# PNP-team/ZPrize23-gpu-submission

Measured on AMD Instinct MI355X. Metric: gen_proof wall-clock (s), HEIGHT=15 Poseidon tree, 1/2/4/8 MI355X + HBM GB/s, lower is better.
Workload: dtype u64

## Files before the change

### zprize23-gpu-submission_amd/csrc/msm.hip

```cpp
#include <algorithm>
#include "msm_internal.h"
#include "ec.cuh"
#include "ec29.cuh"

namespace pnp {

constexpr uint32_t KEY_ZERO = 0xFFFFFFFFu;
template <int C, class E>
__device__ __forceinline__ void digits_of(const Fr &s, int c_rt, int W_rt, int top_sh, E emit) {
    const int c = C > 0 ? C : c_rt;
    const int W = C > 0 ? (255 + C) / C : W_rt;
    const uint32_t NB = 1u << (c - 1);
    uint32_t carry = 0;
    auto digit = [&](int w) {
        const int bit = w * c;
        const int li = bit >> 5, sh = bit & 31;
        uint32_t lo32 = 0, hi32 = 0;
#pragma unroll
        for (int k = 0; k < 8; k++) {
            lo32 = li == k ? s.v[k] : lo32;
            hi32 = li + 1 == k ? s.v[k] : hi32;
        }
        const uint64_t word = lo32 | ((uint64_t)hi32 << 32);
        uint32_t raw = (uint32_t)(word >> sh) & ((1u << c) - 1);
        raw += carry;
        uint32_t key = KEY_ZERO;
        if (raw > NB) {
            const uint32_t mag = (NB << 1) - raw;
            carry = 1;
            if (mag) key = (mag - 1) | 0x80000000u;
        } else {
            carry = 0;
            if (raw) key = (w == W - 1 ? raw << top_sh : raw) - 1;
        }
        emit(w, key);
    };
    if constexpr (C > 0) {
#pragma unroll
        for (int w = 0; w < (255 + C) / C; w++) digit(w);
    } else {
        for (int w = 0; w < W; w++) digit(w);
    }
}
template <class F>
__device__ __forceinline__ void scalar_digits(const uint64_t *scalars, uint64_t i, uint64_t n, int c, int W,
                                              int top_sh, uint32_t *keys, F fn) {
    const Fr s = from_mont(load_fr(scalars, i));
    auto emit = [&](int w, uint32_t key) {
        keys[(uint64_t)w * n + i] = key;
        fn(key);
    };
    if (c == 20 && W == 13)
        digits_of<20>(s, c, W, top_sh, emit);
    else
        digits_of<0>(s, c, W, top_sh, emit);
}
__global__ void k_digits(const uint64_t *scalars, uint64_t n, int c, int W, int top_sh, uint32_t *keys) {
    uint64_t i = blockIdx.x * (uint64_t)blockDim.x + threadIdx.x;
    if (i >= n) return;
    scalar_digits(scalars, i, n, c, W, top_sh, keys, [](uint32_t) {});
}

constexpr int MSM_BATCH_MAX = 16;
struct KeyRows {
    uint64_t n;
    int vstride, off, rows;
    uint32_t id_row0;
    uint64_t id_mul;
    uint64_t id_base = 0;
    int nseg = 0;
    uint64_t seg_off[MSM_BATCH_MAX] = {};
};

#ifndef PNP_SORT_CB
#define PNP_SORT_CB 9
#endif
constexpr int SORT_CB = PNP_SORT_CB;
constexpr int SORT_FB_MAX = 11;
static_assert(SORT_CB >= 1 && SORT_CB <= 12, "PNP_SORT_CB out of range (LDS budget of k_coarse_scatter)");
__device__ __forceinline__ uint64_t cidx(int v, int nv, uint32_t b, int NBc, int wmaj, int ch, int nch) {
    if (wmaj <= 1) return ((uint64_t)v * NBc + b) * nch + ch;
    const uint32_t nbl = (uint32_t)NBc / wmaj;
    return (((uint64_t)(b / nbl) * nv + v) * nbl + b % nbl) * nch + ch;
}

__global__ __launch_bounds__(1024) void k_coarse_hist(const uint32_t *keys, KeyRows kr, int fb,
                                                      int NBc, uint64_t chunk, int nch,
                                                      uint32_t *counts, int wmaj = 1) {
    __shared__ uint32_t hist[1 << SORT_CB];
    const int v = blockIdx.y, ch = blockIdx.x;
    for (int b = threadIdx.x; b < NBc; b += blockDim.x) hist[b] = 0;
    __syncthreads();
    const uint64_t n = kr.n;
    uint64_t lo = (uint64_t)ch * chunk, hi = lo + chunk < n ? lo + chunk : n;
    const uint32_t *kb = keys + ((uint64_t)v * kr.vstride + kr.off) * n;
    const bool vec = ((n | chunk) & 3) == 0;
    for (int r = 0; r < kr.rows; r++) {
        const uint32_t *k = kb + (uint64_t)r * n;
        if (vec) {
            for (uint64_t i = lo + 4 * threadIdx.x; i < hi; i += 4 * blockDim.x) {
                uint4 q = *reinterpret_cast<const uint4 *>(k + i);
                uint32_t w[4] = {q.x, q.y, q.z, q.w};
#pragma unroll
                for (int j = 0; j < 4; j++)
                    if (w[j] != KEY_ZERO) atomicAdd(&hist[(w[j] & 0x7FFFFFFFu) >> fb], 1u);
            }
        } else {
            for (uint64_t i = lo + threadIdx.x; i < hi; i += blockDim.x) {
                uint32_t key = k[i];
                if (key != KEY_ZERO) atomicAdd(&hist[(key & 0x7FFFFFFFu) >> fb], 1u);
            }
        }
    }
    __syncthreads();
    for (int b = threadIdx.x; b < NBc; b += blockDim.x) counts[cidx(v, gridDim.y, b, NBc, wmaj, ch, nch)] = hist[b];
}

struct ScalarPtrs {
    static constexpr int MAX = MSM_BATCH_MAX;
    const uint64_t *p[MAX];
};
__global__ __launch_bounds__(1024) void k_digits_hist(ScalarPtrs sp, uint64_t n, int c, int W, int top_sh, int fb,
                                                      int NBc,
                                                      uint64_t chunk, int nch, uint32_t *keys, uint32_t *counts,
                                                      int wmaj = 1) {
    __shared__ uint32_t hist[1 << SORT_CB];
    const int v = blockIdx.y, ch = blockIdx.x;
    for (int b = threadIdx.x; b < NBc; b += blockDim.x) hist[b] = 0;
    __syncthreads();
    const uint64_t lo = (uint64_t)ch * chunk, hi = lo + chunk < n ? lo + chunk : n;
    uint32_t *kv = keys + (uint64_t)v * W * n;
    for (uint64_t i = lo + threadIdx.x; i < hi; i += blockDim.x)
        scalar_digits(sp.p[v], i, n, c, W, top_sh, kv, [&](uint32_t key) {
            if (key != KEY_ZERO) atomicAdd(&hist[(key & 0x7FFFFFFFu) >> fb], 1u);
        });
    __syncthreads();
    for (int b = threadIdx.x; b < NBc; b += blockDim.x) counts[cidx(v, gridDim.y, b, NBc, wmaj, ch, nch)] = hist[b];
}

__global__ __launch_bounds__(256) void k_scan_tiles(uint32_t *d, uint64_t n, uint32_t *tile_sums) {
    __shared__ uint32_t wsum[4];
    uint64_t base = (uint64_t)blockIdx.x * 1024;
    uint32_t v[4], loc = 0;
    for (int k = 0; k < 4; k++) {
        uint64_t i = base + threadIdx.x * 4 + k;
        v[k] = i < n ? d[i] : 0;
        loc += v[k];
    }
    uint32_t x = loc;
    int lane = threadIdx.x & 63, wv = threadIdx.x >> 6;
    for (int off = 1; off < 64; off <<= 1) {
        uint32_t y = __shfl_up(x, off, 64);
        if (lane >= off) x += y;
    }
    if (lane == 63) wsum[wv] = x;
    __syncthreads();
// ... 346 lines not shown
    const uint32_t d = blockIdx.x;
    auto bin_off = [&](uint64_t gbin) { return offs[gbin * nch]; };
    uint32_t over = 0;
    for (int e = 0; e < W; e++) over |= bin_off((uint64_t)(e + 1) * per_d) - bin_off((uint64_t)e * per_d) > cap;
    uint32_t *h = reinterpret_cast<uint32_t *>(send + (uint64_t)d * slot_recs);
    const uint64_t g0 = (uint64_t)d * per_d;
    if (threadIdx.x == 0) {
        h[0] = SLOT_MAGIC;
        h[1] = bin_off(g0 + per_d) - bin_off(g0);
        h[2] = over;
        h[3] = per_d;
        if (dest_counts) dest_counts[d] = h[1];
    }
    for (uint32_t p = threadIdx.x; p < per_d; p += blockDim.x) h[4 + p] = bin_off(g0 + p + 1) - bin_off(g0 + p);
}

__device__ uint32_t block_scan_1024(uint32_t x, uint32_t &excl, uint32_t *wsum) {
    const int lane = threadIdx.x & 63, wv = threadIdx.x >> 6;
    uint32_t inc = x;
    for (int off = 1; off < 64; off <<= 1) {
        const uint32_t y = __shfl_up(inc, off, 64);
        if (lane >= off) inc += y;
    }
    if (lane == 63) wsum[wv] = inc;
    __syncthreads();
    uint32_t pre = 0, tot = 0;
    for (int j = 0; j < 16; j++) {
        pre += j < wv ? wsum[j] : 0;
        tot += wsum[j];
    }
    excl = pre + inc - x;
    __syncthreads();
    return tot;
}

constexpr int SLOT_W_MAX = 64;
__global__ __launch_bounds__(1024) void k_slot_runs(const uint64_t *recv, int W, uint32_t slot_recs,
                                                    uint32_t hdr_recs, uint32_t per_d, uint32_t cap, uint2 *runs,
                                                    uint32_t *out0, uint32_t *bstart_end, uint32_t *flags) {
    __shared__ uint32_t wsum[16];
    __shared__ uint32_t rcarry[SLOT_W_MAX];
    __shared__ uint32_t bad;
    if (threadIdx.x == 0) bad = 0;
    if (threadIdx.x < (uint32_t)W) rcarry[threadIdx.x] = 0;
    __syncthreads();
    if (threadIdx.x < (uint32_t)W) {
        const uint32_t *h = reinterpret_cast<const uint32_t *>(recv + (uint64_t)threadIdx.x * slot_recs);
        if (h[0] != SLOT_MAGIC || h[3] != per_d || h[2]) atomicOr(&bad, 1u);
    }
    __syncthreads();
    uint32_t carry = 0;
    for (uint32_t p0 = 0; p0 < per_d; p0 += 1024) {
        const uint32_t p = p0 + threadIdx.x;
        uint32_t sum = 0;
        for (int r = 0; r < W; r++) {
            const uint32_t *h = reinterpret_cast<const uint32_t *>(recv + (uint64_t)r * slot_recs);
            const uint32_t c = p < per_d ? h[4 + p] : 0;
            uint32_t pre;
            const uint32_t tot = block_scan_1024(c, pre, wsum);
            const uint32_t st = rcarry[r] + pre;
            const uint32_t len = st >= cap ? 0 : (c < cap - st ? c : cap - st);
            if (p < per_d) runs[(uint64_t)p * W + r] = make_uint2((uint32_t)r * slot_recs + hdr_recs + st, len);
            sum += len;
            __syncthreads();
            if (threadIdx.x == 0) rcarry[r] += tot;
        }
        uint32_t pre;
        const uint32_t tot = block_scan_1024(sum, pre, wsum);
        if (p < per_d) out0[p] = carry + pre;
        carry += tot;
    }
    if (threadIdx.x == 0) {
        out0[per_d] = carry;
        bstart_end[0] = carry;
        flags[0] = bad;
        flags[1] = carry;
    }
}

__device__ __forceinline__ uint32_t bucket_start(const uint32_t *offs, uint64_t u, int nch) {
    return offs[u * nch];
}
__device__ __forceinline__ uint64_t next_bucket(const uint32_t *offs, int nch, uint64_t U, uint64_t a, uint32_t k,
                                                uint32_t &next) {
    uint64_t lo = a, hi = a + 1, step = 1;
    uint32_t vhi = bucket_start(offs, hi, nch);
    while (vhi <= k) {
        lo = hi;
        step <<= 1;
        hi = lo + step < U ? lo + step : U;
        vhi = bucket_start(offs, hi, nch);
    }
    while (hi - lo > 1) {
        const uint64_t m = (lo + hi) >> 1;
        const uint32_t vm = bucket_start(offs, m, nch);
        if (vm <= k) lo = m;
        else hi = m, vhi = vm;
    }
    next = vhi;
    return lo;
}
template <class LoadPt, class StorePt>
__device__ __forceinline__ void segment32(uint64_t t, LoadPt ld, StorePt st, const uint32_t *sorted,
                                          const uint32_t *offs, int nch, uint64_t U, uint32_t S) {
    const uint32_t total = bucket_start(offs, U, nch);
    const uint64_t lo64 = t * S;
    if (lo64 >= total) return;
    const uint32_t lo = (uint32_t)lo64;
    const uint32_t hi = lo + S < total ? lo + S : total;
    uint64_t a = 0, b = U;
    while (b - a > 1) {
        uint64_t m = (a + b) >> 1;
        if (bucket_start(offs, m, nch) <= lo) a = m; else b = m;
    }
    uint64_t cur = a;
    bool first = bucket_start(offs, cur, nch) < lo;
    uint32_t next = bucket_start(offs, cur + 1, nch);
    Xyzz acc = Xyzz::inf();
    for (uint32_t k = lo; k < hi; k++) {
        if (k == next) {
            if (first) st(1, t, acc);
            else st(0, cur, acc);
            first = false;
            acc = Xyzz::inf();
            cur = next_bucket(offs, nch, U, cur + 1, k, next);
        }
        uint32_t e = sorted[k];
        Fq x, y;
        ld(e & 0x7FFFFFFFu, x, y);
        if (e >> 31) y = neg(y);
        acc = madd(acc, x, y);
    }
    if (first) st(1, t, acc);
    else if (next > hi) st(2, t, acc);
    else st(0, cur, acc);
}

__global__ __launch_bounds__(256) void k_accumulate_flat(const uint64_t *points,
                                                         const uint32_t *sorted,
                                                         const uint32_t *offs, int nch, uint64_t U,
                                                         uint32_t S, uint64_t *buckets,
                                                         uint64_t *head, uint64_t *tail) {
    uint64_t t = blockIdx.x * (uint64_t)blockDim.x + threadIdx.x;
    auto ld = [points](uint32_t i, Fq &x, Fq &y) {
        x = load_fq(points + 12ULL * i);
        y = load_fq(points + 12ULL * i + 6);
    };
    auto st = [=](int where, uint64_t i, const Xyzz &p) {
        store_xyzz((where == 0 ? buckets : where == 1 ? head : tail) + 24 * i, p);
    };
    segment32(t, ld, st, sorted, offs, nch, U, S);
}

__device__ __forceinline__ void madd29(Xyzz29 &p, const F29 &x2, const F29 &y2) {
    F29 u2 = mul29(x2, p.zz);
    F29 s2 = mul29(y2, p.zzz);
    F29 P = sub29(u2, p.x, F29_KB);
    F29 R = sub29(s2, p.y, F29_KB);
    F29 pp = sqr29(P);
    F29 ppp = mul29(P, pp);
    F29 q = mul29(p.x, pp);
    F29 x3 = sub29(sub29(sub29(sqr29(R), ppp, F29_KA), q, F29_KA), q, F29_KA);
    F29 y3 = mul2_29(R, sub29(q, x3, F29_KB), p.y, neg29(ppp, F29_KA));
    p.zz = mul29(p.zz, pp);
    p.zzz = mul29(p.zzz, ppp);
    p.x = x3;
    p.y = y3;
}
__device__ __forceinline__ bool store29(uint32_t *dst, const Xyzz29 &p) {
    store_f29(dst, p.x);
    store_f29(dst + 14, p.y);
    store_f29(dst + 28, p.zz);
    store_f29(dst + 42, p.zzz);
    return !zero29(p.zz);
}

#ifndef PNP_ACC_WAVES
#define PNP_ACC_WAVES 3
#endif
#ifndef PNP_PT29
#define PNP_PT29 32
#endif
static constexpr uint64_t PT29 = PNP_PT29;

typedef __attribute__((address_space(3))) void lds_void_t;
typedef __attribute__((address_space(1))) void glob_void_t;
__device__ __forceinline__ void stage_point(const uint32_t *p, uint4 *st) {
#pragma unroll
    for (int c = 0; c < 7; c++)
        __builtin_amdgcn_global_load_lds((glob_void_t *)(p + 4 * c), (lds_void_t *)(st + 64 * c), 16, 0, 0);
}
__device__ __forceinline__ void unstage_point(const uint4 *st, F29 &x, F29 &y) {
    uint32_t w[28];
#pragma unroll
    for (int c = 0; c < 7; c++) {
        const uint4 v = st[64 * c];
        w[4 * c] = v.x;
        w[4 * c + 1] = v.y;
        w[4 * c + 2] = v.z;
        w[4 * c + 3] = v.w;
    }
#pragma unroll
    for (int i = 0; i < 14; i++) {
        x.l[i] = w[i];
        y.l[i] = w[14 + i];
    }
}

__global__ __launch_bounds__(256, PNP_ACC_WAVES) void k_accumulate29(const uint32_t *pts29, const uint32_t *sorted,
                                                      const uint32_t *offs, uint64_t U, uint32_t S,
                                                      uint32_t *buckets, uint32_t *head,
                                                      uint32_t *tail, uint32_t *tailb, uint32_t *redo,
                                                      uint32_t *nredo, uint32_t *tlist) {
    __shared__ uint4 stage[4 * 7 * 64];
    __shared__ uint32_t sidx[4 * 64];
    const uint32_t wv = threadIdx.x >> 6, ln = threadIdx.x & 63;
    uint4 *wave_base = stage + 7 * 64 * wv;
    uint32_t *idx_base = sidx + 64 * wv;
    uint64_t t = blockIdx.x * (uint64_t)blockDim.x + threadIdx.x;
    const uint32_t total = offs[U];
    const uint64_t lo64 = t * S;
    if (lo64 >= total) return;
    const uint32_t lo = (uint32_t)lo64;
    const uint32_t hi = lo + S < total ? lo + S : total;
    uint64_t a = 0, b = U;
    while (b - a > 1) {
        uint64_t m = (a + b) >> 1;
        if (offs[m] <= lo) a = m; else b = m;
    }
    uint64_t cur = a;
    bool first = offs[cur] < lo;
    uint32_t next = offs[cur + 1];
    bool ok = true, fresh = true;
    Xyzz29 acc;
    uint32_t e = sorted[lo];
    stage_point(pts29 + PT29 * (e & 0x7FFFFFFFu), wave_base);
    if (lo + 1 < hi)
        __builtin_amdgcn_global_load_lds((glob_void_t *)(sorted + lo + 1), (lds_void_t *)idx_base, 4, 0, 0);
    for (uint32_t k = lo; k < hi; k++) {
        if (k == next) {
            ok &= store29(first ? head + 56 * t : buckets + 56 * cur, acc);
            first = false;
            fresh = true;
            cur = next_bucket(offs, 1, U, cur + 1, k, next);
        }
        F29 x, y;
        __builtin_amdgcn_s_waitcnt(0x0F70);
        unstage_point(wave_base + ln, x, y);
        const uint32_t en = idx_base[ln];
        __builtin_amdgcn_s_waitcnt(0xC07F);
        const uint32_t ecur = e;
        if (k + 1 < hi) {
            stage_point(pts29 + PT29 * (en & 0x7FFFFFFFu), wave_base);
            if (k + 2 < hi)
                __builtin_amdgcn_global_load_lds((glob_void_t *)(sorted + k + 2), (lds_void_t *)idx_base, 4, 0,
                                                 0);
            e = en;
        }
        if (ecur >> 31) y = neg29(y, F29_KA);
        if (fresh) {
            acc.x = x;
            acc.y = y;
            acc.zz = acc.zzz = const29(F29_ONE);
            fresh = false;
        } else {
            madd29(acc, x, y);
        }
    }
    const bool to_tail = !first && next > hi;
    ok &= store29(first ? head + 56 * t : (to_tail ? tail + 56 * t : buckets + 56 * cur), acc);
    tailb[t] = to_tail ? (uint32_t)cur : NO_TAIL;
    const uint64_t m = __ballot(to_tail);
    if (to_tail) {
        const int leader = __ffsll((unsigned long long)m) - 1;
        const uint32_t below = __builtin_amdgcn_mbcnt_hi((uint32_t)(m >> 32), __builtin_amdgcn_mbcnt_lo((uint32_t)m, 0u));
        uint32_t base = 0;
        if (below == 0) base = atomicAdd(tlist, (uint32_t)__popcll(m));
        base = __shfl(base, leader);
        tlist[1 + base + below] = (uint32_t)t;
    }
    if (!ok) redo[atomicAdd(nredo, 1u)] = (uint32_t)t;
}

constexpr int WCTR_SLOTS = 64;
__global__ __launch_bounds__(1024) void k_count_pieces(const uint32_t *offs, uint64_t WB, uint32_t S,
                                                       unsigned long long *ctr) {
    __shared__ uint32_t part[16];
    const uint64_t b = blockIdx.x * (uint64_t)blockDim.x + threadIdx.x;
    bool fresh = false;
    if (b < WB) {
        const uint32_t o = offs[b];
        fresh = offs[b + 1] > o && (o % S) != 0;
    }
    const unsigned long long m = __ballot(fresh);
    if ((threadIdx.x & 63) == 0) part[threadIdx.x >> 6] = (uint32_t)__popcll(m);
    __syncthreads();
    if (threadIdx.x == 0) {
        uint32_t t = 0;
        for (int w = 0; w < (int)(blockDim.x >> 6); w++) t += part[w];
        if (t) atomicAdd(&ctr[1 + (blockIdx.x & (WCTR_SLOTS - 1))], (unsigned long long)t);
        if (blockIdx.x == 0) {
            const unsigned long long tot = offs[WB];
            ctr[0] = tot;
            atomicAdd(&ctr[1], (tot + S - 1) / S);
        }
    }
}

__global__ __launch_bounds__(64) void k_accumulate_redo(const uint32_t *pts29, const uint32_t *sorted,
                                                        const uint32_t *offs, uint64_t U, uint32_t S,
                                                        uint32_t *buckets, uint32_t *head,
                                                        uint32_t *tail, const uint32_t *redo,
                                                        const uint32_t *nredo) {
    auto ld = [pts29](uint32_t i, Fq &x, Fq &y) {
        x = to_fq32(load29(pts29 + PT29 * i));
        y = to_fq32(load29(pts29 + PT29 * i + 14));
    };
    auto st = [=](int where, uint64_t i, const Xyzz &p) {
        uint32_t *d = (where == 0 ? buckets : where == 1 ? head : tail) + 56 * i;
        store_f29(d, from_fq32(p.x));
        store_f29(d + 14, from_fq32(p.y));
        store_f29(d + 28, from_fq32(p.zz));
        store_f29(d + 42, from_fq32(p.zzz));
    };
    const uint32_t cnt = *nredo;
    for (uint32_t r = blockIdx.x * blockDim.x + threadIdx.x; r < cnt; r += gridDim.x * blockDim.x)
        segment32(redo[r], ld, st, sorted, offs, 1, U, S);
}

__global__ __launch_bounds__(256) void k_table_dbl(const uint64_t *src, uint64_t n, int c,
                                                   uint64_t *xyzz) {
    uint64_t i = blockIdx.x * (uint64_t)blockDim.x + threadIdx.x;
    if (i >= n) return;
    Xyzz29 q;
    q.x = from_fq32(load_fq(src + 12 * i));
    q.y = from_fq32(load_fq(src + 12 * i + 6));
    q.zz = q.zzz = const29(F29_ONE);
#pragma unroll 1
    for (int k = 0; k < c; k++) q = xdbl29(q);
    store_xyzz(xyzz + 24 * i, to32(q));
}
__global__ __launch_bounds__(256) void k_table_affine(const uint64_t *xyzz, uint64_t n, uint32_t CH,
                                                      uint64_t *pre, uint64_t *dst) {
    uint64_t t = blockIdx.x * (uint64_t)blockDim.x + threadIdx.x;
    uint64_t lo = t * CH;
    if (lo >= n) return;
    uint64_t hi = lo + CH < n ? lo + CH : n;
    Fq acc = Fq::one();
    for (uint64_t i = lo; i < hi; i++) {
        Fq z = load_fq(xyzz + 24 * i + 18);
        if (z.is_zero()) z = Fq::one();
        acc = acc * z;
        store_fq(pre + 6 * i, acc);
    }
    Fq inv = inverse(acc);
    for (uint64_t i = hi; i-- > lo;) {
        Fq z = load_fq(xyzz + 24 * i + 18);
        const bool inf = z.is_zero();
        if (inf) z = Fq::one();
        Fq izzz = i > lo ? inv * load_fq(pre + 6 * (i - 1)) : inv;
        inv = inv * z;
        Fq w = load_fq(xyzz + 24 * i + 12) * izzz;
        Fq x = load_fq(xyzz + 24 * i) * (w * w);
        Fq y = load_fq(xyzz + 24 * i + 6) * izzz;
        if (inf) x = y = Fq::zero();
        store_fq(dst + 12 * i, x);
        store_fq(dst + 12 * i + 6, y);
    }
}

__global__ void k_table_to29(const uint64_t *T, uint64_t count, uint32_t *T29) {
    uint64_t i = blockIdx.x * (uint64_t)blockDim.x + threadIdx.x;
    if (i >= count) return;
    F29 x = from_fq32(load_fq(T + 12 * i)), y = from_fq32(load_fq(T + 12 * i + 6));
    uint32_t *o = T29 + PT29 * i;
#pragma unroll
    for (int j = 0; j < 14; j++) {
        o[j] = x.l[j];
        o[14 + j] = y.l[j];
    }
}

void msm_build_table(DevBuf &tab, const uint64_t *d_points, uint64_t n, int c, hipStream_t s) {
    MsmCfg g = msm_cfg(n, c, true);
    const uint64_t count = (uint64_t)g.W * n;
    tab.alloc(count * PT29 * 4);
    uint32_t *T29 = static_cast<uint32_t *>(tab.p);
    const dim3 nb((uint32_t)((n + 255) / 256));
    hipLaunchKernelGGL(k_table_to29, nb, dim3(256), 0, s, d_points, n, T29);
    PNP_HIP(hipGetLastError());
    bg_step(s);
    if (g.W > 1) {
        DevBuf cur(n * 96), nxt(n * 96), xyzz(n * 192), pre(n * 48);
        const uint32_t CH = 64;
        const uint64_t lanes = (n + CH - 1) / CH;
        const uint64_t *src = d_points;
        for (int k = 1; k < g.W; k++) {
            const int dbls = k == g.W - 1 ? g.c - g.top_sh : g.c;
            hipLaunchKernelGGL(k_table_dbl, nb, dim3(256), 0, s, src, n, dbls, xyzz.u64());
            PNP_HIP(hipGetLastError());
            bg_step(s);
            hipLaunchKernelGGL(k_table_affine, dim3((uint32_t)((lanes + 255) / 256)), dim3(256), 0, s,
                               xyzz.u64(), n, CH, pre.u64(), nxt.u64());
            PNP_HIP(hipGetLastError());
            bg_step(s);
            hipLaunchKernelGGL(k_table_to29, nb, dim3(256), 0, s, nxt.u64(), n, T29 + (uint64_t)k * n * PT29);
            PNP_HIP(hipGetLastError());
            bg_step(s);
            std::swap(cur, nxt);
            src = cur.u64();
        }
    }
    PNP_HIP(hipStreamSynchronize(s));
}

void xyzz_to_affine_dev(const uint64_t *xyzz, uint64_t n, uint64_t *aff, hipStream_t s) {
    const uint32_t CH = 64;
    const uint64_t lanes = (n + CH - 1) / CH;
    DevBuf pre(n * 48);
    hipLaunchKernelGGL(k_table_affine, dim3((uint32_t)((lanes + 255) / 256)), dim3(256), 0, s, xyzz, n, CH,
                       pre.u64(), aff);
    PNP_HIP(hipGetLastError());
    PNP_HIP(hipStreamSynchronize(s));
}

static void put_xyzz(const Xyzz &r, uint64_t *o) {
    to_u64_limbs(r.x, o);
    to_u64_limbs(r.y, o + 6);
    to_u64_limbs(r.zz, o + 12);
    to_u64_limbs(r.zzz, o + 18);
}
static Xyzz get_xyzz(const uint64_t *e) {
    Xyzz p;
    p.x = from_u64_limbs<FqP>(e);
    p.y = from_u64_limbs<FqP>(e + 6);
    p.zz = from_u64_limbs<FqP>(e + 12);
    p.zzz = from_u64_limbs<FqP>(e + 18);
    return p;
}

struct GroupPlan {
    KeyRows kr;
    int nv;
};

static void sort_group(MsmWork &wk, MsmGroup &gb, const uint32_t *keys, const GroupPlan &gp,
                       const MsmCfg &g, hipStream_t s, const uint64_t *const *scalars = nullptr) {
    const int nv = gp.nv;
    const uint64_t n = gp.kr.n, WB = (uint64_t)nv * g.NB;
    const int nch0 = std::max(1, 512 / std::max(nv, 1));
    const uint64_t chunk = std::max<uint64_t>(1024, (n + nch0 - 1) / nch0);
    const int nch = (int)((n + chunk - 1) / chunk);
    const int cb = std::min(SORT_CB, g.c - 1), fb = g.c - 1 - cb, NBc = 1 << cb;
    if (fb > SORT_FB_MAX) {
        set_error("msm: window of %d bits exceeds the sort's %d", g.c, SORT_CB + SORT_FB_MAX + 1);
        throw Error(PNP_E_ARG);
    }
    const uint64_t nbins = (uint64_t)nv * NBc;
    const uint64_t nent = (uint64_t)nv * gp.kr.rows * n;
    auto need = [](DevBuf &b, size_t bytes) { if (b.bytes < bytes) b.alloc(bytes); };
    need(gb.counts, (nbins * nch + 1) * 4);
    need(gb.offsets, (WB + 1) * 4);
    need(gb.ent, nent * 4 + 4);
    need(gb.fkey, nent * 2 + 8);
    need(gb.sorted, nent * 4 + 4);
    uint32_t *counts = static_cast<uint32_t *>(gb.counts.p);
    uint32_t *bstart = static_cast<uint32_t *>(gb.offsets.p);
    dim3 grid((uint32_t)nch, (uint32_t)nv);
    if (scalars) {
        ScalarPtrs sp{};
        for (int v = 0; v < nv; v++) sp.p[v] = scalars[v];
        hipLaunchKernelGGL(k_digits_hist, grid, dim3(1024), 0, s, sp, n, g.c, g.W, g.top_sh, fb, NBc, chunk, nch,
                           const_cast<uint32_t *>(keys), counts, 1);
    } else {
        hipLaunchKernelGGL(k_coarse_hist, grid, dim3(1024), 0, s, keys, gp.kr, fb, NBc, chunk, nch, counts);
    }
    PNP_HIP(hipGetLastError());
    const uint64_t ncount = nbins * nch;
    PNP_HIP(hipMemsetAsync(counts + ncount, 0, 4, s));
    scan_u32(counts, ncount + 1, gb.scan_tmp, s);
    uint32_t *ent = static_cast<uint32_t *>(gb.ent.p);
    uint16_t *fk = static_cast<uint16_t *>(gb.fkey.p);
    hipLaunchKernelGGL(k_coarse_scatter, grid, dim3(1024), 0, s, keys, gp.kr, fb, NBc, chunk, nch,
                       counts, ent, fk);
    PNP_HIP(hipGetLastError());
    hipLaunchKernelGGL(k_fine_sort, dim3((uint32_t)nbins), dim3(1024), 0, s, ent, fk, counts, nch, fb,
                       bstart, static_cast<uint32_t *>(gb.sorted.p));
    PNP_HIP(hipGetLastError());
    PNP_HIP(hipMemcpyAsync(bstart + WB, counts + ncount, 4, hipMemcpyDeviceToDevice, s));
}

static uint32_t acc_segment(uint64_t nent, bool folded) {
    uint32_t S = (uint32_t)std::max<uint64_t>(64, (nent >> 20) & ~7ULL);
    if (!folded) return S;
    static uint64_t slots = 0;
    if (!slots) {
        int dev = 0, cus = 0;
        PNP_HIP(hipGetDevice(&dev));
        PNP_HIP(hipDeviceGetAttribute(&cus, hipDeviceAttributeMultiprocessorCount, dev));
        slots = (uint64_t)cus * 4 * PNP_ACC_WAVES * 64;
    }
    const uint64_t per = (nent + slots - 1) / slots;
    const uint64_t rounds = std::max<uint64_t>(1, per / S);
    return (uint32_t)std::max<uint64_t>(16, (per + rounds - 1) / rounds);
}

static void accumulate_group(MsmWork &wk, MsmGroup &gb, const GroupPlan &gp, const MsmCfg &g,
                             const uint64_t *pts, const uint64_t *table, hipStream_t s, uint64_t nent = 0,
                             double alg_bytes = 0) {
    const int nv = gp.nv;
    const uint64_t n = gp.kr.n, WB = (uint64_t)nv * g.NB;
    if (!nent) nent = (uint64_t)nv * gp.kr.rows * n;
    if (alg_bytes == 0) alg_bytes = (double)n * 128.0 * nv * gp.kr.rows / g.W;
    auto need = [](DevBuf &b, size_t bytes) { if (b.bytes < bytes) b.alloc(bytes); };
    need(gb.buckets, (WB * 24 + WB * 72 + 64) * 8);
    const uint32_t *bstart = static_cast<const uint32_t *>(gb.offsets.p);
    const uint32_t *sorted = static_cast<const uint32_t *>(gb.sorted.p);
    uint64_t *bk = gb.buckets.u64();
    hipEvent_t ev0 = nullptr;
    if (wk.timer) wk.timer->begin("msm_accumulate", s, ev0);
    const uint32_t S = acc_segment(nent, table != nullptr);
    const uint64_t nthr = (nent + S - 1) / S;
    if (table) {
        need(gb.seg, (WB + 2 * nthr) * 224 + nthr * 4 + (nthr + 1) * 4);
        uint32_t *bk29 = static_cast<uint32_t *>(gb.seg.p);
        uint32_t *head = bk29 + 56 * WB, *tail = head + 56 * nthr, *tailb = tail + 56 * nthr;
        uint32_t *tlist = tailb + nthr;
        PNP_HIP(hipMemsetAsync(tlist, 0, 4, s));
        need(gb.redo, nthr * 4 + 16);
        uint32_t *nredo = static_cast<uint32_t *>(gb.redo.p), *redo = nredo + 4;
        PNP_HIP(hipMemsetAsync(nredo, 0, 4, s));
        const uint32_t *t29 = reinterpret_cast<const uint32_t *>(table);
// ... 569 lines not shown
```

Baseline: 0.1258.

## Switch MSM bucket accumulation to signed 30-bit limb field arithmetic

```diff
diff --git a/zprize23-gpu-submission_amd/csrc/f30s_consts.inc b/zprize23-gpu-submission_amd/csrc/f30s_consts.inc
--- /dev/null
+++ b/zprize23-gpu-submission_amd/csrc/f30s_consts.inc
@@ -0,0 +1,7 @@
+#pragma once
+__device__ constexpr int32_t F30S_Q[13] = {-21845, -402915328, 356515836, -352321620, -252304353, 55215067, 288093811, 316751073, -321428361, 517541167, -375082566, -91332614, 1704210};
+__device__ constexpr int32_t F30S_QINV = -196611;
+__device__ constexpr int32_t F30S_ONE[13] = {13762350, 433586176, -192935228, -301937177, 37952645, -425753694, -36732706, 162803105, -437337492, 366579475, 78814996, -442511456, 89578};
+__device__ constexpr int32_t F30S_C384[13] = {196605, 405012480, 12582951, -50330895, 123255532, -496935601, -445360651, 370465813, -328370226, -362903204, 154517618, -251748295, 1439327};
+__device__ constexpr int32_t F30S_C396[13] = {-192885889, -32767999, -532500185, -13403472, -35343150, 503405810, 6050829, -194530918, -181768796, 433626394, -273043482, -129447912, 620336};
+__device__ constexpr int32_t F30S_C406[13] = {61471620, 365953864, -372989380, 300627865, -316224671, -47436294, -43116879, -277221202, 12095981, 252526454, -479373662, 205318198, 1257852};
diff --git a/zprize23-gpu-submission_amd/csrc/field30s.cuh b/zprize23-gpu-submission_amd/csrc/field30s.cuh
--- /dev/null
+++ b/zprize23-gpu-submission_amd/csrc/field30s.cuh
@@ -0,0 +1,181 @@
+#pragma once
+#include "field29.cuh"
+#include "f30s_consts.inc"
+
+namespace pnp {
+
+struct F30s {
+    int32_t l[13];
+};
+
+__device__ __forceinline__ int32_t bal30(uint32_t x) { return (int32_t)(x << 2) >> 2; }
+__device__ __forceinline__ int64_t mad30s(int32_t a, int32_t b, int64_t acc) { return acc + (int64_t)a * b; }
+__device__ __forceinline__ int64_t carry30(int64_t acc) { return (acc + (1 << 29)) >> 30; }
+
+__device__ __forceinline__ int64_t reduce_col30s(int k, int64_t acc, int32_t *m, F30s &r) {
+#pragma unroll
+    for (int i = (k > 12 ? k - 12 : 0); i < (k < 13 ? k : 13); i++) acc = mad30s(m[i], F30S_Q[k - i], acc);
+    if (k < 13) {
+        m[k] = bal30((uint32_t)acc * (uint32_t)F30S_QINV);
+        return mad30s(m[k], F30S_Q[0], acc) >> 30;
+    }
+    r.l[k - 13] = bal30((uint32_t)acc);
+    return carry30(acc);
+}
+
+__device__ __forceinline__ F30s mul30s(const F30s &a, const F30s &b) {
+    int32_t m[13];
+    F30s r;
+    int64_t acc = 0;
+#pragma unroll
+    for (int k = 0; k < 25; k++) {
+#pragma unroll
+        for (int i = (k > 12 ? k - 12 : 0); i <= (k < 12 ? k : 12); i++) acc = mad30s(a.l[i], b.l[k - i], acc);
+        acc = reduce_col30s(k, acc, m, r);
+    }
+    r.l[12] = (int32_t)acc;
+    return r;
+}
+
+__device__ __forceinline__ F30s sqr30s(const F30s &a) {
+    int32_t m[13], a2[13];
+#pragma unroll
+    for (int i = 0; i < 13; i++) a2[i] = a.l[i] * 2;
+    F30s r;
+    int64_t acc = 0;
+#pragma unroll
+    for (int k = 0; k < 25; k++) {
+#pragma unroll
+        for (int i = (k > 12 ? k - 12 : 0); 2 * i < k; i++) acc = mad30s(a.l[i], a2[k - i], acc);
+        if ((k & 1) == 0) acc = mad30s(a.l[k / 2], a.l[k / 2], acc);
+        acc = reduce_col30s(k, acc, m, r);
+    }
+    r.l[12] = (int32_t)acc;
+    return r;
+}
+
+__device__ __forceinline__ F30s mul2_30s(const F30s &a, const F30s &b, const F30s &c, const F30s &d) {
+    int32_t m[13];
+    F30s r;
+    int64_t acc = 0;
+#pragma unroll
+    for (int k = 0; k < 25; k++) {
+#pragma unroll
+        for (int i = (k > 12 ? k - 12 : 0); i <= (k < 12 ? k : 12); i++) {
+            acc = mad30s(a.l[i], b.l[k - i], acc);
+            acc = mad30s(c.l[i], d.l[k - i], acc);
+        }
+        if (3 * (k < 13 ? k + 1 : 25 - k) > 31) {
+            const int64_t hi = carry30(acc);
+            acc = reduce_col30s(k, (int64_t)bal30((uint32_t)acc), m, r) + hi;
+        } else {
+            acc = reduce_col30s(k, acc, m, r);
+        }
+    }
+    r.l[12] = (int32_t)acc;
+    return r;
+}
+
+template <bool THREE>
+__device__ __forceinline__ F30s norm30s(const int32_t *t) {
+    F30s r;
+    int32_t c = 0;
+#pragma unroll
+    for (int i = 0; i < 12; i++) {
+        const int32_t s = t[i] + c;
+        r.l[i] = bal30((uint32_t)s);
+        c = THREE ? (s >> 30) + ((s >> 29) & 1) : (s + (1 << 29)) >> 30;
+    }
+    r.l[12] = t[12] + c;
+    return r;
+}
+__device__ __forceinline__ F30s sub30s(const F30s &a, const F30s &b) {
+    int32_t t[13];
+#pragma unroll
+    for (int i = 0; i < 13; i++) t[i] = a.l[i] - b.l[i];
+    return norm30s<false>(t);
+}
+__device__ __forceinline__ F30s sub2_30s(const F30s &a, const F30s &b, const F30s &c) {
+    int32_t t[13];
+#pragma unroll
+    for (int i = 0; i < 13; i++) t[i] = a.l[i] - b.l[i] - c.l[i];
+    return norm30s<true>(t);
+}
+__device__ __forceinline__ F30s neg30s(const F30s &a) {
+    F30s r;
+#pragma unroll
+    for (int i = 0; i < 13; i++) r.l[i] = -a.l[i];
+    return r;
+}
+
+__device__ __forceinline__ F30s const30s(const int32_t *c) {
+    F30s r;
+#pragma unroll
+    for (int i = 0; i < 13; i++) r.l[i] = c[i];
+    return r;
+}
+
+__device__ __forceinline__ void lift30s(const F30s &r, uint32_t *u) {
+    int32_t c = 0;
+#pragma unroll
+    for (int i = 0; i < 12; i++) {
+        const int32_t t = r.l[i] + F30S_Q[i] + c;
+        u[i] = (uint32_t)t & 0x3FFFFFFFu;
+        c = t >> 30;
+    }
+    u[12] = (uint32_t)(r.l[12] + F30S_Q[12] + c);
+}
+
+__device__ __forceinline__ F29 to_f29(const F30s &a) {
+    uint32_t u[13];
+    lift30s(mul30s(a, const30s(F30S_C406)), u);
+    F29 r;
+#pragma unroll
+    for (int j = 0; j < 14; j++) {
+        const int bit = 29 * j, w = bit / 30, sh = bit % 30;
+        uint64_t x = u[w];
+        if (w + 1 < 13) x |= (uint64_t)u[w + 1] << 30;
+        r.l[j] = (uint32_t)(x >> sh) & F29_M;
+    }
+    return r;
+}
+
+__device__ __forceinline__ Fq to_fq32(const F30s &a) {
+    uint32_t u[13];
+    lift30s(mul30s(a, const30s(F30S_C384)), u);
+    Fq r;
+#pragma unroll
+    for (int w = 0; w < 12; w++) {
+        const int bit = 32 * w, j = bit / 30, sh = bit % 30;
+        uint64_t x = (uint64_t)u[j] >> sh;
+        if (j + 1 < 13) x |= (uint64_t)u[j + 1] << (30 - sh);
+        if (j + 2 < 13 && 60 - sh < 32) x |= (uint64_t)u[j + 2] << (60 - sh);
+        r.v[w] = (uint32_t)x;
+    }
+    reduce_once(r);
+    return r;
+}
+
+__device__ __forceinline__ F30s to_f30s(const Fq &a) {
+    F30s t;
+    uint32_t c = 0;
+#pragma unroll
+    for (int j = 0; j < 13; j++) {
+        const int bit = 30 * j, w = bit >> 5, sh = bit & 31;
+        uint64_t x = a.v[w];
+        if (w + 1 < 12) x |= (uint64_t)a.v[w + 1] << 32;
+        const uint32_t u = ((uint32_t)(x >> sh) & 0x3FFFFFFFu) + c;
+        t.l[j] = j < 12 ? bal30(u) : (int32_t)u;
+        c = (u + (1u << 29)) >> 30;
+    }
+    return mul30s(t, const30s(F30S_C396));
+}
+
+__device__ __forceinline__ F30s load30s(const uint32_t *p) {
+    F30s r;
+#pragma unroll
+    for (int i = 0; i < 13; i++) r.l[i] = (int32_t)p[i];
+    return r;
+}
+
+}
diff --git a/zprize23-gpu-submission_amd/csrc/msm.hip b/zprize23-gpu-submission_amd/csrc/msm.hip
--- a/zprize23-gpu-submission_amd/csrc/msm.hip
+++ b/zprize23-gpu-submission_amd/csrc/msm.hip
@@ -2,6 +2,7 @@
 #include "msm_internal.h"
 #include "ec.cuh"
 #include "ec29.cuh"
+#include "field30s.cuh"
 
 namespace pnp {
 
@@ -654,27 +655,62 @@
     segment32(t, ld, st, sorted, offs, nch, U, S);
 }
 
-__device__ __forceinline__ void madd29(Xyzz29 &p, const F29 &x2, const F29 &y2) {
-    F29 u2 = mul29(x2, p.zz);
-    F29 s2 = mul29(y2, p.zzz);
-    F29 P = sub29(u2, p.x, F29_KB);
-    F29 R = sub29(s2, p.y, F29_KB);
-    F29 pp = sqr29(P);
-    F29 ppp = mul29(P, pp);
-    F29 q = mul29(p.x, pp);
-    F29 x3 = sub29(sub29(sub29(sqr29(R), ppp, F29_KA), q, F29_KA), q, F29_KA);
-    F29 y3 = mul2_29(R, sub29(q, x3, F29_KB), p.y, neg29(ppp, F29_KA));
-    p.zz = mul29(p.zz, pp);
-    p.zzz = mul29(p.zzz, ppp);
+struct Xyzz30s {
+    F30s x, y, zz, zzz;
+};
+__device__ __forceinline__ void madd30s(Xyzz30s &p, const F30s &x2, const F30s &y2) {
+    F30s u2 = mul30s(x2, p.zz);
+    F30s s2 = mul30s(y2, p.zzz);
+    F30s P = sub30s(u2, p.x);
+    F30s R = sub30s(s2, p.y);
+    F30s pp = sqr30s(P);
+    F30s ppp = mul30s(P, pp);
+    F30s q = mul30s(p.x, pp);
+    F30s x3 = sub30s(sub2_30s(sqr30s(R), ppp, q), q);
+    F30s y3 = mul2_30s(R, sub30s(q, x3), p.y, neg30s(ppp));
+    p.zz = mul30s(p.zz, pp);
+    p.zzz = mul30s(p.zzz, ppp);
     p.x = x3;
     p.y = y3;
 }
-__device__ __forceinline__ bool store29(uint32_t *dst, const Xyzz29 &p) {
-    store_f29(dst, p.x);
-    store_f29(dst + 14, p.y);
-    store_f29(dst + 28, p.zz);
-    store_f29(dst + 42, p.zzz);
-    return !zero29(p.zz);
+__device__ __forceinline__ void park30s(uint32_t *dst, const Xyzz30s &p) {
+    uint32_t w[52];
+#pragma unroll
+    for (int i = 0; i < 13; i++) {
+        w[i] = (uint32_t)p.x.l[i];
+        w[13 + i] = (uint32_t)p.y.l[i];
+        w[26 + i] = (uint32_t)p.zz.l[i];
+        w[39 + i] = (uint32_t)p.zzz.l[i];
+    }
+    uint4 *q = reinterpret_cast<uint4 *>(dst);
+#pragma unroll
+    for (int c = 0; c < 13; c++) q[c] = make_uint4(w[4 * c], w[4 * c + 1], w[4 * c + 2], w[4 * c + 3]);
+}
+__device__ __forceinline__ bool store29(uint32_t *dst) {
+    uint32_t w[52];
+    const uint4 *q = reinterpret_cast<const uint4 *>(dst);
+#pragma unroll
+    for (int c = 0; c < 13; c++) {
+        const uint4 v = q[c];
+        w[4 * c] = v.x;
+        w[4 * c + 1] = v.y;
+        w[4 * c + 2] = v.z;
+        w[4 * c + 3] = v.w;
+    }
+    Xyzz30s p;
+#pragma unroll
+    for (int i = 0; i < 13; i++) {
+        p.x.l[i] = (int32_t)w[i];
+        p.y.l[i] = (int32_t)w[13 + i];
+        p.zz.l[i] = (int32_t)w[26 + i];
+        p.zzz.l[i] = (int32_t)w[39 + i];
+    }
+    const F29 zz = to_f29(p.zz);
+    store_f29(dst, to_f29(p.x));
+    store_f29(dst + 14, to_f29(p.y));
+    store_f29(dst + 28, zz);
+    store_f29(dst + 42, to_f29(p.zzz));
+    return !zero29(zz);
 }
 
 #ifndef PNP_ACC_WAVES
@@ -692,7 +728,7 @@
     for (int c = 0; c < 7; c++)
         __builtin_amdgcn_global_load_lds((glob_void_t *)(p + 4 * c), (lds_void_t *)(st + 64 * c), 16, 0, 0);
 }
-__device__ __forceinline__ void unstage_point(const uint4 *st, F29 &x, F29 &y) {
+__device__ __forceinline__ void unstage_point(const uint4 *st, F30s &x, F30s &y) {
     uint32_t w[28];
 #pragma unroll
     for (int c = 0; c < 7; c++) {
@@ -703,9 +739,9 @@
         w[4 * c + 3] = v.w;
     }
 #pragma unroll
-    for (int i = 0; i < 14; i++) {
-        x.l[i] = w[i];
-        y.l[i] = w[14 + i];
+    for (int i = 0; i < 13; i++) {
+        x.l[i] = (int32_t)w[i];
+        y.l[i] = (int32_t)w[13 + i];
     }
 }
 
@@ -719,9 +755,9 @@
     const uint32_t wv = threadIdx.x >> 6, ln = threadIdx.x & 63;
     uint4 *wave_base = stage + 7 * 64 * wv;
     uint32_t *idx_base = sidx + 64 * wv;
-    uint64_t t = blockIdx.x * (uint64_t)blockDim.x + threadIdx.x;
+    const uint32_t t = blockIdx.x * blockDim.x + threadIdx.x;
     const uint32_t total = offs[U];
-    const uint64_t lo64 = t * S;
+    const uint64_t lo64 = (uint64_t)t * S;
     if (lo64 >= total) return;
     const uint32_t lo = (uint32_t)lo64;
     const uint32_t hi = lo + S < total ? lo + S : total;
@@ -730,23 +766,23 @@
         uint64_t m = (a + b) >> 1;
         if (offs[m] <= lo) a = m; else b = m;
     }
-    uint64_t cur = a;
+    uint32_t cur = (uint32_t)a;
     bool first = offs[cur] < lo;
     uint32_t next = offs[cur + 1];
     bool ok = true, fresh = true;
-    Xyzz29 acc;
+    Xyzz30s acc;
     uint32_t e = sorted[lo];
     stage_point(pts29 + PT29 * (e & 0x7FFFFFFFu), wave_base);
     if (lo + 1 < hi)
         __builtin_amdgcn_global_load_lds((glob_void_t *)(sorted + lo + 1), (lds_void_t *)idx_base, 4, 0, 0);
     for (uint32_t k = lo; k < hi; k++) {
         if (k == next) {
-            ok &= store29(first ? head + 56 * t : buckets + 56 * cur, acc);
+            park30s((first ? head : buckets) + 56ull * (first ? t : cur), acc);
             first = false;
             fresh = true;
-            cur = next_bucket(offs, 1, U, cur + 1, k, next);
-        }
-        F29 x, y;
+            cur = (uint32_t)next_bucket(offs, 1, U, (uint64_t)cur + 1, k, next);
+        }
+        F30s x, y;
         __builtin_amdgcn_s_waitcnt(0x0F70);
         unstage_point(wave_base + ln, x, y);
         const uint32_t en = idx_base[ln];
@@ -759,19 +795,36 @@
                                                  0);
             e = en;
         }
-        if (ecur >> 31) y = neg29(y, F29_KA);
+        if (ecur >> 31) y = neg30s(y);
         if (fresh) {
             acc.x = x;
             acc.y = y;
-            acc.zz = acc.zzz = const29(F29_ONE);
+            acc.zz = acc.zzz = const30s(F30S_ONE);
             fresh = false;
         } else {
-            madd29(acc, x, y);
+            madd30s(acc, x, y);
         }
     }
     const bool to_tail = !first && next > hi;
-    ok &= store29(first ? head + 56 * t : (to_tail ? tail + 56 * t : buckets + 56 * cur), acc);
-    tailb[t] = to_tail ? (uint32_t)cur : NO_TAIL;
+    park30s(first ? head + 56ull * t : (to_tail ? tail + 56ull * t : buckets + 56ull * cur), acc);
+    tailb[t] = to_tail ? cur : NO_TAIL;
+    {
+        const uint32_t lo2 = t * S;
+        uint64_t c2 = 0, b2 = U;
+        while (b2 - c2 > 1) {
+            uint64_t m = (c2 + b2) >> 1;
+            if (offs[m] <= lo2) c2 = m; else b2 = m;
+        }
+        const uint32_t tot2 = offs[U], hi2 = lo2 + S < tot2 ? lo2 + S : tot2;
+        bool f2 = offs[c2] < lo2;
+        uint32_t n2 = offs[c2 + 1];
+        for (;;) {
+            ok &= store29(f2 ? head + 56ull * t : (n2 > hi2 ? tail + 56ull * t : buckets + 56 * c2));
+            if (n2 >= hi2) break;
+            f2 = false;
+            c2 = next_bucket(offs, 1, U, c2 + 1, n2, n2);
+        }
+    }
     const uint64_t m = __ballot(to_tail);
     if (to_tail) {
         const int leader = __ffsll((unsigned long long)m) - 1;
@@ -779,9 +832,9 @@
         uint32_t base = 0;
         if (below == 0) base = atomicAdd(tlist, (uint32_t)__popcll(m));
         base = __shfl(base, leader);
-        tlist[1 + base + below] = (uint32_t)t;
-    }
-    if (!ok) redo[atomicAdd(nredo, 1u)] = (uint32_t)t;
+        tlist[1 + base + below] = t;
+    }
+    if (!ok) redo[atomicAdd(nredo, 1u)] = t;
 }
 
 constexpr int WCTR_SLOTS = 64;
@@ -815,8 +868,8 @@
                                                         uint32_t *tail, const uint32_t *redo,
                                                         const uint32_t *nredo) {
     auto ld = [pts29](uint32_t i, Fq &x, Fq &y) {
-        x = to_fq32(load29(pts29 + PT29 * i));
-        y = to_fq32(load29(pts29 + PT29 * i + 14));
+        x = to_fq32(load30s(pts29 + PT29 * i));
+        y = to_fq32(load30s(pts29 + PT29 * i + 13));
     };
     auto st = [=](int where, uint64_t i, const Xyzz &p) {
         uint32_t *d = (where == 0 ? buckets : where == 1 ? head : tail) + 56 * i;
@@ -874,12 +927,12 @@
 __global__ void k_table_to29(const uint64_t *T, uint64_t count, uint32_t *T29) {
     uint64_t i = blockIdx.x * (uint64_t)blockDim.x + threadIdx.x;
     if (i >= count) return;
-    F29 x = from_fq32(load_fq(T + 12 * i)), y = from_fq32(load_fq(T + 12 * i + 6));
+    F30s x = to_f30s(load_fq(T + 12 * i)), y = to_f30s(load_fq(T + 12 * i + 6));
     uint32_t *o = T29 + PT29 * i;
 #pragma unroll
-    for (int j = 0; j < 14; j++) {
-        o[j] = x.l[j];
-        o[14 + j] = y.l[j];
+    for (int j = 0; j < 13; j++) {
+        o[j] = (uint32_t)x.l[j];
+        o[13 + j] = (uint32_t)y.l[j];
     }
 }
 
```

Measured after the change: 0.1230, median of 6. -2.2%, faster.
